# thecasterian/fluca

Hardware: AMD Instinct MI355X
Metric: pressure-Poisson Jacobi-PCG iterations/s, 512^3 cells per GPU (higher is better)
Workload: dtype f64

## Files before the change

fluca_amd/csrc/fl_cheb2.hip:

```cpp
#include <type_traits>

#include "fl_device.h"
#include "fl_handle.h"

namespace fl {

typedef double v2d_t __attribute__((ext_vector_type(2)));
template <int NT>
__device__ __forceinline__ double2 c2_ld2(const double *p)
{
  if (NT) {
    const v2d_t v = __builtin_nontemporal_load(reinterpret_cast<const v2d_t *>(p));
    return make_double2(v.x, v.y);
  }
  return *reinterpret_cast<const double2 *>(p);
}
template <int NT>
__device__ __forceinline__ void c2_st2(double *p, double2 v)
{
  if (NT) {
    v2d_t t;
    t.x = v.x;
    t.y = v.y;
    __builtin_nontemporal_store(t, reinterpret_cast<v2d_t *>(p));
// ... 24 lines not shown
}

__device__ __forceinline__ int c2_xcd_remap(int b, int nblocks) { return (nblocks & 7) ? b : (b & 7) * (nblocks >> 3) + (b >> 3); }

template <int RY, int NW, bool JAC, int NT, bool MGD = false, int Z = 0>
__global__ void __launch_bounds__(64 * NW) k_cheb2(GridP g, int perx, int pery, int perz, const double *X0, const double *X1, double *X0w, double *X1w, const double *__restrict__ b, const double *D0, const double *D1, double *D0w,
                                                  double *D1w, const KspScal *__restrict__ s, double *__restrict__ partial, int stride, int zc, int tiles_x, int tiles, int remap, const double *__restrict__ zq = nullptr,
                                                  const double *__restrict__ za_dev = nullptr, double *__restrict__ bw = nullptr)
{
  constexpr bool ZR = Z != 0, ZS = Z == 2;
  static_assert(!(ZR && MGD), "the three-step sweep is the pre-smoother: no sums of the outer iteration");
  constexpr int TX = 128, TY = NW * RY, LX = TX + 4, NTH = 64 * NW;
  constexpr int NTL = NT >= 2, NTS = NT >= 1;
  __shared__ __attribute__((aligned(16))) double XJ[3][TY + 4][LX];
  __shared__ __attribute__((aligned(16))) double XN[3][TY + 2][LX];
  __shared__ double                              red[6 * NW], cB[2 * TY][5];
  if (s->reason != 0) return;

  const double *x  = s->cur ? X1 : X0;
  double       *xn = s->cur ? X0w : X1w;
  const double *d  = s->dcur ? D1 : D0;
  double       *dn = s->dcur ? D0w : D1w;
  double        rho0 = s->cheb_rho, c0 = s->cheb_c;
  double        rho1, c1;
  const double  cf = s->cheb_c;
  const double  za = ZS ? *za_dev : 0.;
  {
    double ck, ckm1;
    cheb_advance(s, s->ck, s->ckm1, ck, ckm1, rho1, c1);
    if (ZR) {
      rho0 = rho1;
      c0   = c1;
      double ck2, ckm2;
      cheb_advance(s, ck, ckm1, ck2, ckm2, rho1, c1);
    }
  }

  const int bb    = remap ? c2_xcd_remap(blockIdx.x, gridDim.x) : blockIdx.x;
  const int chunk = bb / tiles, tile = bb % tiles;
  const int i0 = (tile % tiles_x) * TX, j0 = (tile / tiles_x) * TY;
// ... 140 lines not shown
        R.hxB = c2_LD1(hx, HB.off);
        R.hbB = c2_LD1(hb, HB.off);
        R.hdB = c2_LD1(hd, HB.off);
      }
      if (anyE) R.hxE = c2_LD1(hx, HE.off);
    }
    R.zcw = ZR ? g.sc[2][pk] : 0.;
    R.pl  = pl;
    const int kz = min(max(kk, -1), g.nz);
    R.zl  = g.sl[2][kz];
    R.zc  = g.sc[2][kz];
    R.zh  = g.sh[2][kz];
    R.pin = pin;
  };

  double  acc[6] = {0., 0., 0., 0., 0., 0.};
  double2 sb2[RY], d1p[RY];
  double2 zb1[RY], zb1R = make_double2(0., 0.);
  double  zb1B = 0.;
  double  z1l = 0., z1c = 0., z1h = 0., z2l = 0., z2c = 0., z2h = 0.;
  bool    pin1 = false;
#pragma unroll
  for (int m = 0; m < RY; ++m) sb2[m] = d1p[m] = zb1[m] = make_double2(0., 0.);

  auto step = [&](auto do1, auto do2, int kk, Raw &C, Raw &N) {
    constexpr bool DO1 = decltype(do1)::value, DO2 = decltype(do2)::value;
    load(kk + 1, N);
    double2 zbn[RY], zbnR = make_double2(0., 0.);
    double  zbnB = 0.;
    if constexpr (ZR) {
      const bool ownk = kk >= k0 && kk < k1;
// ... 99 lines not shown
      if (anyB) {
        const double cen = XJ[bc][HB.lr][HB.lc], dyz = cB[tbc][4] + z1c;
        const double v = dyz * cen + cB[tbc][0] * XJ[bc][HB.lr][HB.lc - 1] + cB[tbc][1] * XJ[bc][HB.lr][HB.lc + 1] + cB[tbc][2] * XJ[bc][HB.lr - 1][HB.lc] + cB[tbc][3] * XJ[bc][HB.lr + 1][HB.lc] + z1l * XJ[bp][HB.lr][HB.lc] + z1h * C.hxB;
        const double r = (ZR ? zb1B : C.hbB) - v, z = JAC ? r / dyz : r;
        const double e = (rho0 != 0. ? rho0 * (ZR ? cen : C.hdB) : 0.) + c0 * z;
        hx1B = (HB.in && pin1) ? cen + e : 0.;
      }
    }

    if constexpr (DO2) {
      const int     bc = (k2 + 3) % 3, bp = (k2 + 2) % 3;
      const int64_t p2 = (int64_t)k2 * g.sxy;
#pragma unroll
      for (int m = 0; m < RY; ++m) {
        const int     lr    = w * RY + m + 1;
        const double2 cen   = *reinterpret_cast<const double2 *>(&XN[bc][lr][lc]);
        const double2 south = *reinterpret_cast<const double2 *>(&XN[bc][lr - 1][lc]);
        const double2 north = *reinterpret_cast<const double2 *>(&XN[bc][lr + 1][lc]);
        const double2 below = *reinterpret_cast<const double2 *>(&XN[bp][lr][lc]);
        const double  west = XN[bc][lr][lc - 1], east = XN[bc][lr][lc + 2];
        const double  dyz = yc[m] + z2c;
        const double  v0 = (xc0 + dyz) * cen.x + xl0 * west + xh0 * cen.y + yl[m] * south.x + yh[m] * north.x + z2l * below.x + z2h * x1v[m].x;
        const double  v1 = (xc1 + dyz) * cen.y + xl1 * cen.x + xh1 * east + yl[m] * south.y + yh[m] * north.y + z2l * below.y + z2h * x1v[m].y;
        const double  r0 = sb2[m].x - v0, r1 = sb2[m].y - v1;
        const double  z0 = JAC ? r0 / (xc0 + dyz) : r0, z1 = JAC ? r1 / (xc1 + dyz) : r1;
        double2       e, xo;
        e.x  = rho1 * d1p[m].x + c1 * z0;
        e.y  = rho1 * d1p[m].y + c1 * z1;
        xo.x = cen.x + e.x;
        xo.y = cen.y + e.y;
        if (rin[m] && in0) {
          if (in1) {
            c2_ST2<NTS>(dn + rob[m] + p2, lo, e);
            c2_ST2<NTS>(xn + rob[m] + p2, lo, xo);
            if (MGD) {
              acc[0] += xo.x + xo.y;
              acc[1] += xo.x * xo.x + xo.y * xo.y;
              acc[2] += sb2[m].x * xo.x + sb2[m].y * xo.y;
              acc[3] += sb2[m].x + sb2[m].y;
              acc[4] += sb2[m].x * sb2[m].x + sb2[m].y * sb2[m].y;
            } else {
              acc[3] += z0 + z1;
              acc[4] += z0 * z0 + z1 * z1;
              acc[5] += r0 * r0 + r1 * r1;
            }
          } else {
            c2_ST1(dn + rob[m] + p2, lo, e.x);
            c2_ST1(xn + rob[m] + p2, lo, xo.x);
            if (MGD) {
              acc[0] += xo.x;
              acc[1] += xo.x * xo.x;
              acc[2] += sb2[m].x * xo.x;
              acc[3] += sb2[m].x;
              acc[4] += sb2[m].x * sb2[m].x;
            } else {
              acc[3] += z0;
              acc[4] += z0 * z0;
              acc[5] += r0 * r0;
            }
          }
        }
      }
    }

    {
      const int bj = (kk + 3) % 3, bn = (kc + 3) % 3;
#pragma unroll
      for (int m = 0; m < RY; ++m) {
        if (rin[m]) {
// ... 46 lines not shown
    using F = std::false_type;
    Raw A, B;
    __syncthreads();
    load(k0 - 2, A);
    step(F(), F(), k0 - 2, A, B);
    step(F(), F(), k0 - 1, B, A);
    step(T(), F(), k0, A, B);
    step(T(), F(), k0 + 1, B, A);
    for (int kk = k0 + 2; kk <= k1 + 1; kk += 2) {
      step(T(), T(), kk, A, B);
      if (kk + 1 <= k1 + 1) step(T(), T(), kk + 1, B, A);
    }
  }

#pragma unroll
  for (int a = 0; a < 6; ++a) {
    acc[a] = wave_sum(acc[a]);
    if (lane == 0) red[a * NW + w] = acc[a];
  }
  __syncthreads();
  if (tid == 0) {
#pragma unroll
    for (int a = 0; a < 6; ++a) {
      double t = 0.;
#pragma unroll
      for (int q = 0; q < NW; ++q) t += red[a * NW + q];
      partial[(int64_t)a * stride + blockIdx.x] = t;
    }
  }
}

}

using namespace fl;


bool fl_cheb2_usable(const fl_poisson *h)
{
// ... 59 lines not shown
    } else {
      if (jac) cheb2_t<4, true, false, 2>(h, p, X0, X1, B, D0, D1, subq, suba_dev, Bw);
      else cheb2_t<4, false, false, 2>(h, p, X0, X1, B, D0, D1, subq, suba_dev, Bw);
    }
    return;
  }
  if (p.nw == 8) {
    if (jac) cheb2_t<8, true, false, 1>(h, p, X0, X1, B, D0, D1);
    else cheb2_t<8, false, false, 1>(h, p, X0, X1, B, D0, D1);
  } else {
    if (jac) cheb2_t<4, true, false, 1>(h, p, X0, X1, B, D0, D1);
    else cheb2_t<4, false, false, 1>(h, p, X0, X1, B, D0, D1);
  }
}

void fl_launch_cheb2(fl_poisson *h, const Cheb2Plan &p, bool jac, double *X0, double *X1, const double *B, double *D0, double *D1, bool mgdots)
{
  if (mgdots) {
    if (p.nw == 8) cheb2_t<8, true, true>(h, p, X0, X1, B, D0, D1);
    else cheb2_t<4, true, true>(h, p, X0, X1, B, D0, D1);
    return;
  }
  if (p.nw == 8) {
    if (jac) cheb2_t<8, true>(h, p, X0, X1, B, D0, D1);
    else cheb2_t<8, false>(h, p, X0, X1, B, D0, D1);
  } else {
    if (jac) cheb2_t<4, true>(h, p, X0, X1, B, D0, D1);
    else cheb2_t<4, false>(h, p, X0, X1, B, D0, D1);
  }
}
```

fluca_amd/csrc/fl_handle.h:

```cpp
#pragma once
#include <algorithm>
#include <cmath>
#include <cstdlib>
#include <cstring>
#include <limits>
#include <list>
#include <string>

#include "fl_internal.h"
#include "fl_knobs.h"

typedef struct ncclComm *ncclComm_t;

namespace fl {

void launch_pad_copy(hipStream_t, const GridP &, const double *, double *);
void launch_unpad_copy(hipStream_t, const GridP &, const double *, double *, const double *);
void launch_project_all(hipStream_t, const GridP &, const double *p, double *const v[3], double *const V[3]);
bool project_six_usable(const GridP &, const double *p_unpadded, double *const v[3], double *const V[3]);
void launch_project_six(hipStream_t, const GridP &, const double *p, bool direct, int per, double *const v[3], double *const V[3]);
void launch_wrap(hipStream_t, const GridP &, double *, int axis, int nvec = 1, int64_t vstride = 0);
void launch_pack_faces_sr(hipStream_t, const GridP &, const double *r, const double *sb, const double *W, const KspScal *s, double *const bufs[6]);
void launch_face_ext(hipStream_t, const GridP &, double *v, double *buf, int axis, int side, int ea, int eb, int mode);
void launch_face_ext_deep(hipStream_t, const GridP &, double *v, double *buf, int axis, int side, int ea, int eb, int dp, int mode);
// ... 74 lines not shown
  int  exchange(hipStream_t st, const std::vector<Msg> &m);
  int  allreduce(hipStream_t st, double *dev, int n);
  void destroy_oneshot();
  void destroy();
};

}

using namespace fl;


struct fl_mg;

struct SmoothSeq {
  int                  nu = 0;
  bool                 guess_zero = false, jac = false, fuse = false, want = false, zero3 = false;
  double               emin = 0., emax = 0.;
  std::vector<KspScal> host;
  KspScal             *dev = nullptr;
};

struct fl_poisson {
  int         device = 0;
  hipStream_t stream = nullptr, own_stream = nullptr;
  Axis        ax[3];
  int         bc[6];
  double      kappa = 0.;
  fl_decomp   dec;
  int         nbr[6];
  bool        wrap_local[3];
  bool        multi = false;
// ... 101 lines not shown
int  fl_fill_ghosts_deep(fl_poisson *h, double *v);
int  fl_fill_hifaces(fl_poisson *h, const double *const V[3]);
int  fl_exchange_r_begin(fl_poisson *h, double *r, const double *q);
int  fl_exchange_sr_begin(fl_poisson *h, const double *r, const double *sb, const double *W, double *rn);
int  fl_exchange_r_end(fl_poisson *h, double *r);
bool fl_any_ghost_exchange(const fl_poisson *h);
int fl_allreduce_max(fl_poisson *h, double *v);
int fl_allreduce_sum(fl_poisson *h, double *v);
int fl_poll_scal(fl_poisson *h);
int fl_apply_tiled(fl_poisson *h, const double *xpad, double *y, int unpadded_y);
int fl_residual(fl_poisson *h, const double *x, const double *b, double *r);
int fl_residual_padded(fl_poisson *h, double *xpad, const double *bpad, double *rpad);
bool fl_residual_restrict_fusable(const GridP &g);
int fl_residual_restrict_padded(fl_poisson *h, double *xpad, const double *bpad, const double *wx, const double *wy, const double *wz, fl_poisson *hc, double *cpad);
int fl_apply_padded_dot(fl_poisson *h, double *xpad, double *ypad, double *xy);
int fl_cheb_smooth_padded(fl_poisson *h, int nu, bool jac, bool guess_zero, bool *mgdots = nullptr, const double *subq = nullptr, const double *suba_dev = nullptr);
int fl_solve_cg(fl_poisson *h, const double *b, double *x, const fl_ksp_opts *o, fl_ksp_stats *st);
int fl_solve_bcgs(fl_poisson *h, const double *b, double *x, const fl_ksp_opts *o, fl_ksp_stats *st);
int fl_solve_cg_sr(fl_poisson *h, const double *b, double *x, const fl_ksp_opts *o, fl_ksp_stats *st);
int fl_ksp_begin(fl_poisson *h, const fl_ksp_opts *o);
int fl_bcgs_fin_step(fl_poisson *h, int mode, int nblocks, int nslot, int nhist);
int fl_ksp_finish(fl_poisson *h, const fl_ksp_opts *o, fl_ksp_stats *st);
int fl_cheb_begin(fl_poisson *h, const fl_ksp_opts *o, double emin, double emax);
int fl_cheb_fin_step(fl_poisson *h, int nblocks, int nhist);
int fl_solve_cheb(fl_poisson *h, const double *b, double *x, const fl_ksp_opts *o, fl_ksp_stats *st);
double fl_gershgorin_bound(const fl_poisson *h, bool jac);
struct Cheb2Plan {
  int nw, tiles_x, tiles, nchunk, zc, nblocks;
};
bool      fl_cheb2_usable(const fl_poisson *h);
int       fl_cheb2_agree(fl_poisson *h);
Cheb2Plan fl_cheb2_plan(const GridP &g);
void      fl_launch_cheb2(fl_poisson *h, const Cheb2Plan &p, bool jac, double *X0, double *X1, const double *B, double *D0, double *D1, bool mgdots = false);
namespace fl {
struct SchurVarT {
  const double *w0[3], *w1[3];
  const int    *c0[3];
};
}
bool      fl_schur_var_usable(const fl_poisson *h);
int       fl_schur_var_fill_ghosts(fl_poisson *h, double *p_pad);
int       fl_schur_var_apply_fused(fl_poisson *h, const fl::SchurVarT &t, const double *ainv, const double *p_pad, double *y);
struct SchurVarPlan {
  int     per_xcd, nseg, band, fixed_seg;
  int64_t items;
};
SchurVarPlan schur_var_plan(const fl::GridP &g);
struct TP {
// ... 8 lines not shown
```

fluca_amd/csrc/fl_internal.h:

```cpp
#pragma once
#include <hip/hip_runtime.h>

#include <algorithm>
#include <cstdint>
#include <cstdio>
#include <vector>

#include "../../include/fluca_hip.h"

#define FL_HIP(call)                                                                                          \
  do {                                                                                                        \
    hipError_t e_ = (call);                                                                                   \
    if (e_ != hipSuccess) {                                                                                   \
      std::fprintf(stderr, "[flucahip] %s:%d %s -> %s\n", __FILE__, __LINE__, #call, hipGetErrorString(e_)); \
      return FL_ERR_GPU;                                                                                      \
    }                                                                                                         \
  } while (0)

#define FL_CHK(call)          \
  do {                        \
    int rc_ = (call);         \
    if (rc_ != 0) return rc_; \
  } while (0)

// ... 56 lines not shown
  R.v[1]    = P1;
  return R;
}

struct KspScal {
  double rz, rz_old, pq, alpha, beta, zshift, dp, rnorm0, ttol;
  double aring[CG_XRING_MAX];
  double rtol, atol, dtol;
  double ncell_global;
  double rho, rho_old, omega, omega_old, d1, d2, vshift, tshift, rshift;
  double ck, ckm1, mu, omegaprod, scale, xshift, dshift, cheb_rho, cheb_c;
  int    it, maxit, reason, norm_type, nullspace, pending_x, cur;
  int    x_valid;
  int    dcur;
  int    xdepth;
};

constexpr int MAX_PARTIAL_BLOCKS = 4096;
constexpr int NSLOT              = 8;

inline int z_chunk_count(int tiles, int nz, int target_blocks, int min_zc = 8)
{
  const int nchunk = std::min(std::max(1, (target_blocks + tiles / 2) / tiles), std::max(1, nz / min_zc));
  return std::max(1, std::min(nchunk, nz));
}
struct ZChunks {
  int nchunk, zc;
};
inline ZChunks z_chunks(int nz, int nchunk)
{
// ... 21 lines not shown
```

fluca_amd/csrc/fl_knobs.h:

```cpp
#pragma once
#include <atomic>

#define FL_PUBLIC_KNOBS(X)                                                                                                                   \
  X(cheb_fuse, 1)                   \
  X(placement, 0)                           \
  X(cg_xbatch, 1)                                           \
  X(cg_xdepth, 8)                 \
  X(cheb_zero3, 1)                  \
  X(mg_prolong, 1)                                                             \
  X(mg_flexible, 1)                                                             \
  X(mg_coarse, 1)                                   \
  X(mg_post_smooth, 0)               \
  X(schur_var_fused, 1)      \
  X(overlap, 1)              \
  X(comm_loopback, 0)           \
  X(comm_trace, 0)                             \
  X(ghost_width, 0)                                       \
  X(placement_verbose, 0)                                                                        \
  X(placement_vmm, 1)                    \
  X(allreduce, 0)

namespace fl {

enum Knob : int {
#define X(n, d) K_##n,
  FL_PUBLIC_KNOBS(X)
#undef X
// ... 10 lines not shown
```

fluca_amd/csrc/fl_ksp.hip:

```cpp
#include <ctime>
#include "fl_handle.h"
#include "fl_device.h"
#include "fl_stencil.h"

namespace fl {

__device__ __forceinline__ double2 LD2(const double *base, unsigned byteoff) { return *reinterpret_cast<const double2 *>(reinterpret_cast<const char *>(base) + byteoff); }
__device__ __forceinline__ void    ST2(double *base, unsigned byteoff, double2 v) { *reinterpret_cast<double2 *>(reinterpret_cast<char *>(base) + byteoff) = v; }
__device__ __forceinline__ void    ST1(double *base, unsigned byteoff, double v) { *reinterpret_cast<double *>(reinterpret_cast<char *>(base) + byteoff) = v; }
__device__ __forceinline__ double uniform(double v)
{
  const int lo = __builtin_amdgcn_readfirstlane(__double2loint(v)), hi = __builtin_amdgcn_readfirstlane(__double2hiint(v));
  return __hiloint2double(hi, lo);
}


struct Tile {
  int  i, il, k0, k1, lane, w, j0w, i0;
  bool own0, own1;
};
template <int RY>
__device__ __forceinline__ Tile make_tile(const GridP &g, int nchunk, int zc, int tiles_x)
{
  Tile      t;
// ... 194 lines not shown
  static constexpr int NACC = MODE == 9 ? 7 : 4;
  static constexpr bool ZST = MODE == 9 || MODE == 10;
};
template <int RY, int NW, bool JAC, int MODE>
__device__ __forceinline__ void st_body(const GridP &g, const double *__restrict__ stg, const double *e0, const double *e1, const double *e2, double *w0, double *w1 ,
                                        const KspScal *__restrict__ s, double *__restrict__ partial, int stride, int nchunk, int zc, int tiles_x, int tiles, int remap, StAux ax = StAux())
{
  static_assert(MODE != 11 || RY == 2, "the restricted residual pairs the two rows of a wave");
  using T               = TileA<RY, NW>;
  constexpr int TX = T::TX, TY = T::TY, LX = T::LX, LY = T::LY;
  constexpr int NE = BcgsIo<MODE>::NE, NACC = BcgsIo<MODE>::NACC;
  constexpr bool ZST = BcgsIo<MODE>::ZST;
  __shared__ __attribute__((aligned(16))) double lds[3][LY][LX];
  __shared__ double                              red[NACC * NW];
  double alpha = 0., omega = 0., beta = 0., ob = 0., vsh = 0., ssh = 0., tsh = 0., crho = 0., cc = 0., zsh = 0.;
  if (MODE < 7 || MODE == 9 || MODE == 10) {
    if (s->reason != 0) return;
    alpha = s->alpha; omega = s->omega; beta = s->beta; ob = s->omega_old * s->beta; vsh = s->vshift; ssh = s->rshift; tsh = s->tshift;
    crho = s->cheb_rho; cc = s->cheb_c; zsh = s->zshift;
  }

  const int b     = remap ? xcd_remap(blockIdx.x, gridDim.x) : blockIdx.x;
  const int chunk = b / tiles, tile = b % tiles;
  const int i0 = (tile % tiles_x) * TX, j0 = (tile / tiles_x) * TY;
  const int k0 = chunk * zc, k1 = min(k0 + zc, g.nz);
  const int tid = threadIdx.x, lane = tid & 63;
  const int w  = __builtin_amdgcn_readfirstlane(tid >> 6);
  const int i  = i0 + 2 * lane;
  const int jb = j0 + w * RY;

  const bool   own0 = i < g.nx, own1 = i + 1 < g.nx;
  const int    il  = min(i, g.nx & ~1);
  const int    ic0 = min(i, g.nx), ic1 = min(i + 1, g.nx);
  const double xl0 = g.sl[0][ic0], xc0 = g.sc[0][ic0], xh0 = g.sh[0][ic0];
// ... 169 lines not shown
          const double  wyz = e2[min(jb + m, g.ny - 1)] * reinterpret_cast<const double *>(w1)[kc];
          racc += wyz * (rwx0 * (ov.x - y.x) + rwx1 * (ov.y - y.y));
          if (m == RY - 1 && (kc & 1)) {
            if (o1) w0[ax.coff + (int64_t)(kc >> 1) * ax.csxy + (int64_t)(jb >> 1) * ax.csx + (i >> 1)] = racc;
            racc = 0.;
          }
        } else if (MODE == 6) {
          const double2 bv = C.e[0][m], dv = C.e[NE >= 2 ? 1 : 0][m];
          const double  r0 = bv.x - y.x, r1 = bv.y - y.y;
          const double  z0 = JAC ? r0 / (xc0 + dyc) : r0, z1 = JAC ? r1 / (xc1 + dyc) : r1;
          double2       dn, xo;
          dn.x = (crho != 0. ? crho * dv.x : 0.) + cc * z0;
          dn.y = (crho != 0. ? crho * dv.y : 0.) + cc * z1;
          xo.x = cen.x + dn.x;
          xo.y = cen.y + dn.y;
          put(w1, dn);
          put(w0, xo);
          acc[0] += (o0 ? z0 : 0.) + (o1 ? z1 : 0.);
          acc[1] += (o0 ? z0 * z0 : 0.) + (o1 ? z1 * z1 : 0.);
          acc[2] += (o0 ? r0 * r0 : 0.) + (o1 ? r1 * r1 : 0.);
        } else {
          const double2 R = C.e[0][m];
          double2       o;
          o.x = R.x - ob * (y.x - vsh) + beta * cen.x;
          o.y = R.y - ob * (y.y - vsh) + beta * cen.y;
          put(w0, o);
        }
      }
    }
#pragma unroll
    for (int m = 0; m < RY; ++m) {
// ... 172 lines not shown
  s->pq     = dpi;
  s->beta   = b;
  s->alpha  = betan / dpi;
}

template <int RY, bool JAC>
__global__ void __launch_bounds__(256) k_cheb(GridP g, const double *X0, const double *X1, double *X0w, double *X1w, const double *__restrict__ b, double *D0, double *D1,
                                              const KspScal *__restrict__ s, double *__restrict__ partial, int stride, int nchunk, int zc, int tiles_x)
{
  __shared__ double red[3 * 4];
  if (s->reason != 0) return;
  const double *x  = s->cur ? X1 : X0;
  double       *xn = s->cur ? X0w : X1w;
  double *__restrict__ d = s->dcur ? D1 : D0;
  const double  rho = s->cheb_rho, cc = s->cheb_c;
  const Tile    t = make_tile<RY>(g, nchunk, zc, tiles_x);
  const double  xl0 = g.sl[0][min(t.i, g.nx)], xc0 = g.sc[0][min(t.i, g.nx)], xh0 = g.sh[0][min(t.i, g.nx)];
  const double  xl1 = g.sl[0][min(t.i + 1, g.nx)], xc1 = g.sc[0][min(t.i + 1, g.nx)], xh1 = g.sh[0][min(t.i + 1, g.nx)];
  double        acc[3] = {0., 0., 0.};
  if (t.k0 < t.k1) {
    double2       prev[RY], cur[RY], nxt[RY], so_c, no_c, so_n, no_n;
    double        we_c[RY], ee_c[RY], we_n[RY], ee_n[RY];
    unsigned      lo = 8u * (unsigned)t.il;
    const int     i0 = t.i0;
    const int64_t sxy = g.sxy;
    const int64_t rsou = g.off0 + (int64_t)min(t.j0w - 1, g.ny) * g.sx, rnor = g.off0 + (int64_t)min(t.j0w + RY, g.ny) * g.sx;
    int64_t       rj[RY];
#pragma unroll
    for (int m = 0; m < RY; ++m) rj[m] = g.off0 + (int64_t)min(t.j0w + m, g.ny) * g.sx;
    const int wofs = i0 - 1, eofs = min(i0 + 128, g.nx);
// ... 33 lines not shown
        const double  west = t.lane == 0 ? we_c[m] : up, east = t.lane == 63 ? ee_c[m] : dn;
        const double  dyz = ycc + zcc;
        double2       v;
        v.x = (xc0 + dyz) * cur[m].x + xl0 * west + xh0 * cur[m].y + yl * so.x + yh * no.x + zl * prev[m].x + zh * nxt[m].x;
        v.y = (xc1 + dyz) * cur[m].y + xl1 * cur[m].x + xh1 * east + yl * so.y + yh * no.y + zl * prev[m].y + zh * nxt[m].y;
        if (j < g.ny && t.own0) {
          const bool   two = t.own1;
          const double r0 = bv[m].x - v.x, r1 = two ? bv[m].y - v.y : 0.;
          const double z0 = JAC ? r0 / (xc0 + dyz) : r0, z1 = two ? (JAC ? r1 / (xc1 + dyz) : r1) : 0.;
          double2      dn2, xo;
          dn2.x = (rho != 0. ? rho * dv[m].x : 0.) + cc * z0;
          dn2.y = (rho != 0. ? rho * dv[m].y : 0.) + cc * z1;
          xo.x  = cur[m].x + dn2.x;
          xo.y  = cur[m].y + dn2.y;
          if (two) {
            ST2(d + rj[m] + pc, lo, dn2);
            ST2(xn + rj[m] + pc, lo, xo);
          } else {
            ST1(d + rj[m] + pc, lo, dn2.x);
            ST1(xn + rj[m] + pc, lo, xo.x);
          }
          acc[0] += z0 + z1;
          acc[1] += z0 * z0 + z1 * z1;
          acc[2] += r0 * r0 + r1 * r1;
        }
      }
#pragma unroll
      for (int m = 0; m < RY; ++m) {
        prev[m] = cur[m];
        cur[m]  = nxt[m];
        we_c[m] = uniform(we_n[m]);
        ee_c[m] = uniform(ee_n[m]);
      }
      so_c = so_n;
// ... 366 lines not shown

int fl_apply_padded_dot(fl_poisson *h, double *xpad, double *ypad, double *xy)
{
  FL_CHK(fl_fill_ghosts(h, xpad));
  const PlanA pa = plan_cg_A(h->g, 0, 0);
  FL_CHK(fl_ensure_partials(h, pa.nblocks));
  launch_bcgs_st<7>(h, pa, false, xpad, nullptr, nullptr, nullptr, ypad, nullptr);
  launch_reduce(h->stream, h->partial, pa.nblocks, h->partial_stride, 4, h->sums);
  if (h->multi) FL_CHK(h->comm.allreduce(h->stream, h->sums, NSLOT));
  if (!xy) return 0;
  FL_HIP(hipMemcpyAsync(xy, h->sums + 2, sizeof(double), hipMemcpyDeviceToHost, h->stream));
  FL_HIP(hipStreamSynchronize(h->stream));
  return 0;
}

int fl_cheb_smooth_padded(fl_poisson *h, int nu, bool jac, bool guess_zero, bool *mgdots, const double *subq, const double *suba)
{
  if (subq && !(guess_zero && nu > 0)) return FL_ERR_ARG_WRONGSTATE;
  const bool want = mgdots && *mgdots;
  if (mgdots) *mgdots = false;
  for (double **v : {&h->r, &h->P0, &h->q, &h->xp}) FL_CHK(fl_ensure_vec(h, v));
  if (nu <= 0) {
    if (guess_zero) FL_CHK(fl_zero_vec(h, h->xp));
    return 0;
  }
  const TP tp = tile_plan(h->g);
  FL_CHK(fl_ensure_partials(h, std::max(tp.nblocks, 1024)));
  const int nhist = nu + 2;
  FL_CHK(fl_ensure_hist(h, nhist));
  hipStream_t  s = h->stream;
  fl_ksp_opts  o;
// ... 23 lines not shown
  }
  double    *X0 = h->xp, *X1 = h->P0, *B = h->r, *D0 = h->q, *D1 = fuse ? h->cd1 : h->q;
  const bool ghosts = fl_any_ghost_exchange(h);
  int        cur = 0, dcur = 0;
  const int trace = knob(K_comm_trace);
  auto mark = [&](const char *what, int j) {
    if (!trace) return;
    const bool sync = trace >= 2;
    const hipError_t e = sync ? hipStreamSynchronize(s) : hipSuccess;
    struct timespec ts;
    clock_gettime(CLOCK_MONOTONIC, &ts);
    std::fprintf(stderr, "[%.3f smooth r%d n=%dx%dx%d] %s j=%d cur=%d dcur=%d -> %s\n", ts.tv_sec % 1000 + 1e-9 * ts.tv_nsec, h->comm.rank, h->g.nx, h->g.ny, h->g.nz, what, j, cur, dcur, hipGetErrorString(e));
    std::fflush(stderr);
  };
  const bool zero3 = fuse && guess_zero && nu >= 3 && !h->multi && knob(K_cheb_zero3) != 0;
  auto kind_of = [&](int j) { return (j == 0 && guess_zero) ? (zero3 ? 3 : 1) : ((fuse && j + 2 <= nu && !(want && jac && !h->multi && ((nu - j) & 1))) ? 2 : 0); };
  const KspScal *seq = nullptr;
  {
    SmoothSeq *hit = nullptr;
    for (SmoothSeq &q : h->smooth_seq)
      if (q.nu == nu && q.guess_zero == guess_zero && q.jac == jac && q.fuse == fuse && q.want == want && q.zero3 == zero3 && q.emin == emin && q.emax == emax) hit = &q;
    if (!hit) {
      SmoothSeq q;
      q.nu = nu; q.guess_zero = guess_zero; q.jac = jac; q.fuse = fuse; q.want = want; q.zero3 = zero3; q.emin = emin; q.emax = emax;
      KspScal S = S0;
      auto advance = [](const KspScal &P, double ck, double ckm1, double &ck_out, double &ckm1_out, double &rho, double &c) {
        const double ckp1 = 2. * P.mu * ck - ckm1, omega = P.omegaprod * ck / ckp1;
        ckm1_out = ck;
        ck_out   = ckp1;
        rho      = omega - 1.;
        c        = omega * P.scale;
      };
      for (int j = 0; j < nu;) {
        q.host.push_back(S);
        if (kind_of(j) == 3) {
          double ck, ckm1, ck2, ckm2, rho, c;
          advance(S, S.ck, S.ckm1, ck, ckm1, rho, c);
          advance(S, ck, ckm1, ck2, ckm2, rho, c);
          S.cur ^= 1;
// ... 11 lines not shown
          S.cheb_rho = rho2;
          S.cheb_c   = c2;
          j += 2;
        } else {
          double ck, ckm1, rho, c;
          S.cur ^= 1;
          S.it += 1;
          advance(S, S.ck, S.ckm1, ck, ckm1, rho, c);
          S.ck       = ck;
          S.ckm1     = ckm1;
          S.cheb_rho = rho;
          S.cheb_c   = c;
          j += 1;
        }
      }
      FL_HIP(hipMalloc((void **)&q.dev, sizeof(KspScal) * q.host.size()));
      h->smooth_seq.push_back(std::move(q));
      hit = &h->smooth_seq.back();
      FL_HIP(hipMemcpyAsync(hit->dev, hit->host.data(), sizeof(KspScal) * hit->host.size(), hipMemcpyHostToDevice, s));
    }
    seq = hit->dev;
  }
  struct ScalGuard {
    fl_poisson *h;
    KspScal    *keep;
    ~ScalGuard() { h->scal = keep; }
  } guard{h, h->scal};
  const bool deep = fuse && h->multi;
  bool       bghost = false;
  int        launch = 0;
// ... 19 lines not shown
      if (subq) {
        if (jac) hipLaunchKernelGGL((k_cheb_first<true, true>), dim3(nb), dim3(256), 0, s, h->g, X0, X1, B, D0, D1, h->scal, subq, suba);
        else hipLaunchKernelGGL((k_cheb_first<false, true>), dim3(nb), dim3(256), 0, s, h->g, X0, X1, B, D0, D1, h->scal, subq, suba);
      } else if (jac) hipLaunchKernelGGL((k_cheb_first<true>), dim3(nb), dim3(256), 0, s, h->g, X0, X1, B, D0, D1, h->scal, (const double *)nullptr, (const double *)nullptr);
      else hipLaunchKernelGGL((k_cheb_first<false>), dim3(nb), dim3(256), 0, s, h->g, X0, X1, B, D0, D1, h->scal, (const double *)nullptr, (const double *)nullptr);
      j += 1;
    } else if (kind == 2) {
      const bool md = want && jac && j + 2 == nu && !h->multi;
      if (deep) {
        if (!bghost) FL_CHK(fl_fill_ghosts(h, B));
        bghost = true;
        FL_CHK(fl_fill_ghosts_deep(h, cur ? X1 : X0));
        FL_CHK(fl_fill_ghosts(h, dcur ? D1 : D0));
      }
      mark("ghosts filled, before fused", j);
      fl_launch_cheb2(h, cp, jac, X0, X1, B, D0, D1, md);
      mark("fused done", j);
      dcur ^= 1;
      if (md) {
        launch_reduce(s, h->partial, cp.nblocks, h->partial_stride, 5, h->sums);
        *mgdots = true;
      }
      j += 2;
    } else {
      if (ghosts) FL_CHK(fl_fill_ghosts(h, cur ? X1 : X0));
      mark("before single", j);
      (void)launch_cheb(h, tp, jac, X0, X1, B, D0, D1);
      mark("single done", j);
      j += 1;
    }
    cur ^= 1;
  }
  if (cur) std::swap(h->xp, h->P0);
  h->poisoned = true;
  return 0;
// ... 323 lines not shown
```

fluca_amd/csrc/fl_mg.hip:

```cpp
#include <new>

#include "fl_handle.h"
#include "fl_device.h"

namespace fl {

struct Owned {
  int64_t npair_row, npairs;
};
__device__ __forceinline__ Owned owned_of(const GridP &g)
{
  Owned o;
  o.npair_row = (g.nx + 1) / 2;
  o.npairs    = o.npair_row * (int64_t)g.ny * g.nz;
  return o;
}
__device__ __forceinline__ int64_t pair_off(const GridP &g, const Owned &o, int64_t q, bool &two)
{
  const int     ip = (int)(q % o.npair_row);
  const int64_t row = q / o.npair_row;
  const int     j = (int)(row % g.ny), k = (int)(row / g.ny);
  two = 2 * ip + 1 < g.nx;
  return g.off0 + (int64_t)k * g.sxy + (int64_t)j * g.sx + 2 * ip;
}
// ... 537 lines not shown
    for (double **v : {&hl->r, &hl->P0, &hl->q, &hl->xp}) FL_CHK(fl_ensure_vec(hl, v));
    if (l + 1 == mg->lv.size()) {
      FL_CHK(alloc_cells(hl, &L.x));
      FL_CHK(alloc_cells(hl, &L.b));
    }
    FL_CHK(fl_ensure_partials(hl, MG_BLOCKS));
  }
  for (double **v : {&h->w0, &h->w1, &h->w2}) FL_CHK(fl_ensure_vec(h, v));
  FL_HIP(hipMalloc((void **)&mg->scal, sizeof(MgScal)));
  FL_HIP(hipMalloc((void **)&mg->slot_dev, 2 * sizeof(MgSlot)));
  FL_HIP(hipHostMalloc((void **)&mg->slot_host, 2 * sizeof(MgSlot)));
  for (hipEvent_t &e : mg->ev_slot) FL_HIP(hipEventCreateWithFlags(&e, hipEventDisableTiming));
  return 0;
}

int vcycle(fl_mg *mg, size_t l, const fl_ksp_opts *o, bool *sums = nullptr, const double *subq = nullptr)
{
  const bool want = sums && *sums;
  if (sums) *sums = false;
  MgLevel    &L = mg->lv[l];
  fl_poisson *h = L.h;
  if (l + 1 == mg->lv.size()) {
    fl_ksp_stats st;
    fl_ksp_opts  so;
    fl_ksp_opts_default(&so);
    so.remove_nullspace = o->remove_nullspace;
    so.type  = FL_KSP_CG;
    so.pc    = FL_PC_JACOBI;
    so.rtol  = 1e-2;
    so.maxit = 200;
    if (subq) hipLaunchKernelGGL(k_mg_pwd<5>, dim3(nblk_pairs(h->g)), dim3(256), 0, h->stream, h->g, (const MgScal *)mg->scal, (const double *)nullptr, subq, (double *)nullptr, h->r);
// ... 32 lines not shown
      t.pn[d] = L.pn[d];
      t.pw[d] = L.pw[d];
    }
    if (L.r[0] == 2 && L.r[1] == 2 && L.r[2] == 2) {
      const int  kc = 4;
      const GridP &gcs = C.h->g;
      hipLaunchKernelGGL(k_mg_prolong_lin_cc, dim3((gcs.nx + 61) / 62, (gcs.ny + 3) / 4, (gcs.nz + kc - 1) / kc), dim3(256), 0, h->stream, h->g, gcs, t, (const double *)C.h->xp, h->xp, kc);
    } else {
      const int  zc = 8;
      const dim3 grid((h->g.nx + 127) / 128, (h->g.ny + 3) / 4, (h->g.nz + zc - 1) / zc);
      hipLaunchKernelGGL(k_mg_prolong_lin_tile, grid, dim3(256), 0, h->stream, h->g, C.h->g, L.r[0], L.r[1], L.r[2], t, (const double *)C.h->xp, h->xp, zc);
    }
  } else hipLaunchKernelGGL(k_mg_prolong_add, dim3(nblk_pairs(h->g)), dim3(256), 0, h->stream, h->g, C.h->g, L.r[0], L.r[1], L.r[2], C.h->xp, h->xp);
  bool got = want;
  const int nu_post = knob(K_mg_post_smooth) > 0 ? knob(K_mg_post_smooth) : nu;
  FL_CHK(fl_cheb_smooth_padded(h, nu_post, true, false, &got));
  if (sums) *sums = got;
  return 0;
}

}

void fl_mg_destroy(fl_poisson *h)
{
  fl_mg *mg = h->mg;
  if (!mg) return;
  for (size_t l = 0; l < mg->lv.size(); ++l) {
    MgLevel &L = mg->lv[l];
    for (double *p : {L.x, L.b, L.w[0], L.w[1], L.w[2], L.pw[0], L.pw[1], L.pw[2]})
      if (p) (void)hipFree(p);
    for (int *p : L.pn)
// ... 53 lines not shown
    MgScal init;
    std::memset(&init, 0, sizeof(init));
    init.N      = N;
    init.ns     = ns ? 1 : 0;
    init.pnorm  = pnorm ? 1 : 0;
    init.rz_old = 1.;
    hipLaunchKernelGGL(k_mg_scal_set, dim3(1), dim3(1), 0, s, S, init);
  }
  auto dots_dev = [&](const double *z, const double *r) -> int {
    hipLaunchKernelGGL(k_mg_dots, dim3(nb), dim3(256), 0, s, g, z, r, h->partial, h->partial_stride);
    launch_reduce(s, h->partial, nb, h->partial_stride, 5, h->sums);
    if (h->multi) FL_CHK(h->comm.allreduce(s, h->sums, NSLOT));
    return 0;
  };
  const double *subq = nullptr;
  auto cycle_and_sums = [&](int it, bool first) -> int {
    bool got = true;
    FL_CHK(vcycle(mg, 0, o, &got, subq));
    if (!got) FL_CHK(dots_dev(h->xp, h->r));
    const int a = it & 1;
    if (first) hipLaunchKernelGGL((k_mg_scal<1, true>), dim3(1), dim3(1), 0, s, S, (const double *)h->sums, mg->slot_dev + a);
    else hipLaunchKernelGGL((k_mg_scal<1, false>), dim3(1), dim3(1), 0, s, S, (const double *)h->sums, mg->slot_dev + a);
    FL_HIP(hipMemcpyAsync(mg->slot_host + a, mg->slot_dev + a, sizeof(MgSlot), hipMemcpyDeviceToHost, s));
    FL_HIP(hipEventRecord(mg->ev_slot[a], s));
    return 0;
  };
  auto look = [&](int it) -> int {
    const int a = it & 1;
    FL_HIP(hipEventSynchronize(mg->ev_slot[a]));
    const MgSlot &L = mg->slot_host[a];
    dp     = L.dp;
    rz     = L.rz;
    pq     = L.pq;
// ... 4 lines not shown
  FL_CHK(fl_zero_vec(h, X));
  FL_CHK(cycle_and_sums(0, true));
  hipLaunchKernelGGL(k_mg_pwd<2>, dim3(nb), dim3(256), 0, s, g, (const MgScal *)S, (const double *)h->xp, (const double *)nullptr, P, (double *)nullptr);
  FL_CHK(look(0));
  const double rnorm0 = dp, ttol = std::max(o->rtol * dp, o->atol);
  hist.push_back(dp);
  int  it = 0, reason = 0;
  auto converged = [&](double v) {
    if (std::isnan(v) || std::isinf(v)) return (int)FL_DIVERGED_NANORINF;
    if (v <= ttol) return v < o->atol ? (int)FL_CONVERGED_ATOL : (int)FL_CONVERGED_RTOL;
    if (v >= o->dtol * rnorm0) return (int)FL_DIVERGED_DTOL;
    return 0;
  };
  reason = converged(dp);
  if (!reason && o->maxit <= 0) reason = FL_DIVERGED_ITS;
  const bool flexible = fl_mg_flexible_mode() != 0;
  while (!reason) {
    FL_CHK(fl_apply_padded_dot(h, P, Q, nullptr));
    hipLaunchKernelGGL((k_mg_scal<0>), dim3(1), dim3(1), 0, s, S, (const double *)h->sums, (MgSlot *)nullptr);
    subq = Q;
    FL_CHK(cycle_and_sums(it + 1, false));
    subq = nullptr;
    if (flexible) {
      FL_CHK(dots_dev(h->xp, Q));
      hipLaunchKernelGGL((k_mg_scal<2>), dim3(1), dim3(1), 0, s, S, (const double *)h->sums, (MgSlot *)nullptr);
    } else hipLaunchKernelGGL((k_mg_scal<3>), dim3(1), dim3(1), 0, s, S, (const double *)h->sums, (MgSlot *)nullptr);
    hipLaunchKernelGGL(k_mg_pwd<4>, dim3(nb), dim3(256), 0, s, g, (const MgScal *)S, (const double *)h->xp, (const double *)nullptr, P, X);
    FL_CHK(look(it + 1));
    if (bad_pq) {
      reason = std::isnan(pq) ? FL_DIVERGED_NANORINF : FL_DIVERGED_INDEFINITE_MAT;
      break;
    }
    ++it;
    hist.push_back(dp);
    reason = converged(dp);
    if (!reason && it >= o->maxit) reason = FL_DIVERGED_ITS;
    if (!reason && !(rz > 0.)) reason = std::isnan(rz) ? FL_DIVERGED_NANORINF : FL_DIVERGED_INDEFINITE_PC;
  }
// ... 30 lines not shown
```

Measured before the change: 715.0.

## Fuse flexible-PCG q·z dots into final smoother sweep and skip dead direction store

The last fused Chebyshev post-smoothing sweep now also reads Q and accumulates q·x and sum(q), so the flexible outer PCG can take its extra dot products from the smoother's reduction. This removes a separate dots kernel and reduce pass over two full vectors each iteration. The final smoother step also skips writing the Chebyshev direction vector when it will not be reused, saving one full-grid store. In exchange the sweep does an additional streaming load of Q and reduces two more accumulators.

```diff
diff --git a/fluca_amd/csrc/fl_cheb2.hip b/fluca_amd/csrc/fl_cheb2.hip
--- a/fluca_amd/csrc/fl_cheb2.hip
+++ b/fluca_amd/csrc/fl_cheb2.hip
@@ -62,7 +62,8 @@
   constexpr int NTL = NT >= 2, NTS = NT >= 1;
   __shared__ __attribute__((aligned(16))) double XJ[3][TY + 4][LX];
   __shared__ __attribute__((aligned(16))) double XN[3][TY + 2][LX];
-  __shared__ double                              red[6 * NW], cB[2 * TY][5];
+  constexpr int NA = MGD ? 7 : 6;
+  __shared__ double                              red[NA * NW], cB[2 * TY][5];
   if (s->reason != 0) return;
 
   const double *x  = s->cur ? X1 : X0;
@@ -72,6 +73,7 @@
   double        rho0 = s->cheb_rho, c0 = s->cheb_c;
   double        rho1, c1;
   const double  cf = s->cheb_c;
+  const bool    keepd = s->d_dead == 0;
   const double  za = ZS ? *za_dev : 0.;
   {
     double ck, ckm1;
@@ -242,7 +244,7 @@
     R.pin = pin;
   };
 
-  double  acc[6] = {0., 0., 0., 0., 0., 0.};
+  double  acc[7] = {0., 0., 0., 0., 0., 0., 0.};
   double2 sb2[RY], d1p[RY];
   double2 zb1[RY], zb1R = make_double2(0., 0.);
   double  zb1B = 0.;
@@ -372,6 +374,7 @@
 #pragma unroll
       for (int m = 0; m < RY; ++m) {
         const int     lr    = w * RY + m + 1;
+        const double2 qv = (MGD && zq) ? c2_LD2<NTL>(zq + rob[m] + p2, lo) : make_double2(0., 0.);
         const double2 cen   = *reinterpret_cast<const double2 *>(&XN[bc][lr][lc]);
         const double2 south = *reinterpret_cast<const double2 *>(&XN[bc][lr - 1][lc]);
         const double2 north = *reinterpret_cast<const double2 *>(&XN[bc][lr + 1][lc]);
@@ -389,7 +392,7 @@
         xo.y = cen.y + e.y;
         if (rin[m] && in0) {
           if (in1) {
-            c2_ST2<NTS>(dn + rob[m] + p2, lo, e);
+            if (keepd) c2_ST2<NTS>(dn + rob[m] + p2, lo, e);
             c2_ST2<NTS>(xn + rob[m] + p2, lo, xo);
             if (MGD) {
               acc[0] += xo.x + xo.y;
@@ -397,13 +400,15 @@
               acc[2] += sb2[m].x * xo.x + sb2[m].y * xo.y;
               acc[3] += sb2[m].x + sb2[m].y;
               acc[4] += sb2[m].x * sb2[m].x + sb2[m].y * sb2[m].y;
+              acc[5] += qv.x * xo.x + qv.y * xo.y;
+              acc[6] += qv.x + qv.y;
             } else {
               acc[3] += z0 + z1;
               acc[4] += z0 * z0 + z1 * z1;
               acc[5] += r0 * r0 + r1 * r1;
             }
           } else {
-            c2_ST1(dn + rob[m] + p2, lo, e.x);
+            if (keepd) c2_ST1(dn + rob[m] + p2, lo, e.x);
             c2_ST1(xn + rob[m] + p2, lo, xo.x);
             if (MGD) {
               acc[0] += xo.x;
@@ -411,6 +416,8 @@
               acc[2] += sb2[m].x * xo.x;
               acc[3] += sb2[m].x;
               acc[4] += sb2[m].x * sb2[m].x;
+              acc[5] += qv.x * xo.x;
+              acc[6] += qv.x;
             } else {
               acc[3] += z0;
               acc[4] += z0 * z0;
@@ -487,14 +494,14 @@
   }
 
 #pragma unroll
-  for (int a = 0; a < 6; ++a) {
+  for (int a = 0; a < NA; ++a) {
     acc[a] = wave_sum(acc[a]);
     if (lane == 0) red[a * NW + w] = acc[a];
   }
   __syncthreads();
   if (tid == 0) {
 #pragma unroll
-    for (int a = 0; a < 6; ++a) {
+    for (int a = 0; a < NA; ++a) {
       double t = 0.;
 #pragma unroll
       for (int q = 0; q < NW; ++q) t += red[a * NW + q];
@@ -584,11 +591,11 @@
   }
 }
 
-void fl_launch_cheb2(fl_poisson *h, const Cheb2Plan &p, bool jac, double *X0, double *X1, const double *B, double *D0, double *D1, bool mgdots)
+void fl_launch_cheb2(fl_poisson *h, const Cheb2Plan &p, bool jac, double *X0, double *X1, const double *B, double *D0, double *D1, bool mgdots, const double *dotq)
 {
   if (mgdots) {
-    if (p.nw == 8) cheb2_t<8, true, true>(h, p, X0, X1, B, D0, D1);
-    else cheb2_t<4, true, true>(h, p, X0, X1, B, D0, D1);
+    if (p.nw == 8) cheb2_t<8, true, true>(h, p, X0, X1, B, D0, D1, dotq);
+    else cheb2_t<4, true, true>(h, p, X0, X1, B, D0, D1, dotq);
     return;
   }
   if (p.nw == 8) {
diff --git a/fluca_amd/csrc/fl_handle.h b/fluca_amd/csrc/fl_handle.h
--- a/fluca_amd/csrc/fl_handle.h
+++ b/fluca_amd/csrc/fl_handle.h
@@ -112,7 +112,7 @@
 
 struct SmoothSeq {
   int                  nu = 0;
-  bool                 guess_zero = false, jac = false, fuse = false, want = false, zero3 = false;
+  bool                 guess_zero = false, jac = false, fuse = false, want = false, zero3 = false, keep_d = false;
   double               emin = 0., emax = 0.;
   std::vector<KspScal> host;
   KspScal             *dev = nullptr;
@@ -244,7 +244,7 @@
 bool fl_residual_restrict_fusable(const GridP &g);
 int fl_residual_restrict_padded(fl_poisson *h, double *xpad, const double *bpad, const double *wx, const double *wy, const double *wz, fl_poisson *hc, double *cpad);
 int fl_apply_padded_dot(fl_poisson *h, double *xpad, double *ypad, double *xy);
-int fl_cheb_smooth_padded(fl_poisson *h, int nu, bool jac, bool guess_zero, bool *mgdots = nullptr, const double *subq = nullptr, const double *suba_dev = nullptr);
+int fl_cheb_smooth_padded(fl_poisson *h, int nu, bool jac, bool guess_zero, bool *mgdots = nullptr, const double *subq = nullptr, const double *suba_dev = nullptr, const double *dotq = nullptr);
 int fl_solve_cg(fl_poisson *h, const double *b, double *x, const fl_ksp_opts *o, fl_ksp_stats *st);
 int fl_solve_bcgs(fl_poisson *h, const double *b, double *x, const fl_ksp_opts *o, fl_ksp_stats *st);
 int fl_solve_cg_sr(fl_poisson *h, const double *b, double *x, const fl_ksp_opts *o, fl_ksp_stats *st);
@@ -261,7 +261,7 @@
 bool      fl_cheb2_usable(const fl_poisson *h);
 int       fl_cheb2_agree(fl_poisson *h);
 Cheb2Plan fl_cheb2_plan(const GridP &g);
-void      fl_launch_cheb2(fl_poisson *h, const Cheb2Plan &p, bool jac, double *X0, double *X1, const double *B, double *D0, double *D1, bool mgdots = false);
+void      fl_launch_cheb2(fl_poisson *h, const Cheb2Plan &p, bool jac, double *X0, double *X1, const double *B, double *D0, double *D1, bool mgdots = false, const double *dotq = nullptr);
 namespace fl {
 struct SchurVarT {
   const double *w0[3], *w1[3];
diff --git a/fluca_amd/csrc/fl_internal.h b/fluca_amd/csrc/fl_internal.h
--- a/fluca_amd/csrc/fl_internal.h
+++ b/fluca_amd/csrc/fl_internal.h
@@ -94,6 +94,7 @@
   int    x_valid;
   int    dcur;
   int    xdepth;
+  int    d_dead;
 };
 
 constexpr int MAX_PARTIAL_BLOCKS = 4096;
diff --git a/fluca_amd/csrc/fl_knobs.h b/fluca_amd/csrc/fl_knobs.h
--- a/fluca_amd/csrc/fl_knobs.h
+++ b/fluca_amd/csrc/fl_knobs.h
@@ -11,6 +11,8 @@
   X(mg_flexible, 1)                                                             \
   X(mg_coarse, 1)                                   \
   X(mg_post_smooth, 0)               \
+  X(smooth_keep_d, 0)        \
+  X(mg_outer_fused, 1)     \
   X(schur_var_fused, 1)      \
   X(overlap, 1)              \
   X(comm_loopback, 0)           \
diff --git a/fluca_amd/csrc/fl_ksp.hip b/fluca_amd/csrc/fl_ksp.hip
--- a/fluca_amd/csrc/fl_ksp.hip
+++ b/fluca_amd/csrc/fl_ksp.hip
@@ -232,10 +232,12 @@
   __shared__ __attribute__((aligned(16))) double lds[3][LY][LX];
   __shared__ double                              red[NACC * NW];
   double alpha = 0., omega = 0., beta = 0., ob = 0., vsh = 0., ssh = 0., tsh = 0., crho = 0., cc = 0., zsh = 0.;
+  bool   keepd = true;
   if (MODE < 7 || MODE == 9 || MODE == 10) {
     if (s->reason != 0) return;
     alpha = s->alpha; omega = s->omega; beta = s->beta; ob = s->omega_old * s->beta; vsh = s->vshift; ssh = s->rshift; tsh = s->tshift;
     crho = s->cheb_rho; cc = s->cheb_c; zsh = s->zshift;
+    if (MODE == 6) keepd = s->d_dead == 0;
   }
 
   const int b     = remap ? xcd_remap(blockIdx.x, gridDim.x) : blockIdx.x;
@@ -435,7 +437,7 @@
           dn.y = (crho != 0. ? crho * dv.y : 0.) + cc * z1;
           xo.x = cen.x + dn.x;
           xo.y = cen.y + dn.y;
-          put(w1, dn);
+          if (keepd) put(w1, dn);
           put(w0, xo);
           acc[0] += (o0 ? z0 : 0.) + (o1 ? z1 : 0.);
           acc[1] += (o0 ? z0 * z0 : 0.) + (o1 ? z1 * z1 : 0.);
@@ -638,6 +640,7 @@
   double       *xn = s->cur ? X0w : X1w;
   double *__restrict__ d = s->dcur ? D1 : D0;
   const double  rho = s->cheb_rho, cc = s->cheb_c;
+  const bool    keepd = s->d_dead == 0;
   const Tile    t = make_tile<RY>(g, nchunk, zc, tiles_x);
   const double  xl0 = g.sl[0][min(t.i, g.nx)], xc0 = g.sc[0][min(t.i, g.nx)], xh0 = g.sh[0][min(t.i, g.nx)];
   const double  xl1 = g.sl[0][min(t.i + 1, g.nx)], xc1 = g.sc[0][min(t.i + 1, g.nx)], xh1 = g.sh[0][min(t.i + 1, g.nx)];
@@ -701,10 +704,10 @@
           xo.x  = cur[m].x + dn2.x;
           xo.y  = cur[m].y + dn2.y;
           if (two) {
-            ST2(d + rj[m] + pc, lo, dn2);
+            if (keepd) ST2(d + rj[m] + pc, lo, dn2);
             ST2(xn + rj[m] + pc, lo, xo);
           } else {
-            ST1(d + rj[m] + pc, lo, dn2.x);
+            if (keepd) ST1(d + rj[m] + pc, lo, dn2.x);
             ST1(xn + rj[m] + pc, lo, xo.x);
           }
           acc[0] += z0 + z1;
@@ -1101,7 +1104,7 @@
   return 0;
 }
 
-int fl_cheb_smooth_padded(fl_poisson *h, int nu, bool jac, bool guess_zero, bool *mgdots, const double *subq, const double *suba)
+int fl_cheb_smooth_padded(fl_poisson *h, int nu, bool jac, bool guess_zero, bool *mgdots, const double *subq, const double *suba, const double *dotq)
 {
   if (subq && !(guess_zero && nu > 0)) return FL_ERR_ARG_WRONGSTATE;
   const bool want = mgdots && *mgdots;
@@ -1155,15 +1158,16 @@
     std::fflush(stderr);
   };
   const bool zero3 = fuse && guess_zero && nu >= 3 && !h->multi && knob(K_cheb_zero3) != 0;
+  const bool keep_d = knob(K_smooth_keep_d) != 0;
   auto kind_of = [&](int j) { return (j == 0 && guess_zero) ? (zero3 ? 3 : 1) : ((fuse && j + 2 <= nu && !(want && jac && !h->multi && ((nu - j) & 1))) ? 2 : 0); };
   const KspScal *seq = nullptr;
   {
     SmoothSeq *hit = nullptr;
     for (SmoothSeq &q : h->smooth_seq)
-      if (q.nu == nu && q.guess_zero == guess_zero && q.jac == jac && q.fuse == fuse && q.want == want && q.zero3 == zero3 && q.emin == emin && q.emax == emax) hit = &q;
+      if (q.nu == nu && q.guess_zero == guess_zero && q.jac == jac && q.fuse == fuse && q.want == want && q.zero3 == zero3 && q.keep_d == keep_d && q.emin == emin && q.emax == emax) hit = &q;
     if (!hit) {
       SmoothSeq q;
-      q.nu = nu; q.guess_zero = guess_zero; q.jac = jac; q.fuse = fuse; q.want = want; q.zero3 = zero3; q.emin = emin; q.emax = emax;
+      q.nu = nu; q.guess_zero = guess_zero; q.jac = jac; q.fuse = fuse; q.want = want; q.zero3 = zero3; q.keep_d = keep_d; q.emin = emin; q.emax = emax;
       KspScal S = S0;
       auto advance = [](const KspScal &P, double ck, double ckm1, double &ck_out, double &ckm1_out, double &rho, double &c) {
         const double ckp1 = 2. * P.mu * ck - ckm1, omega = P.omegaprod * ck / ckp1;
@@ -1205,6 +1209,7 @@
           j += 1;
         }
       }
+      q.host.back().d_dead = keep_d ? 0 : 1;
       FL_HIP(hipMalloc((void **)&q.dev, sizeof(KspScal) * q.host.size()));
       h->smooth_seq.push_back(std::move(q));
       hit = &h->smooth_seq.back();
@@ -1254,11 +1259,11 @@
         FL_CHK(fl_fill_ghosts(h, dcur ? D1 : D0));
       }
       mark("ghosts filled, before fused", j);
-      fl_launch_cheb2(h, cp, jac, X0, X1, B, D0, D1, md);
+      fl_launch_cheb2(h, cp, jac, X0, X1, B, D0, D1, md, md ? dotq : nullptr);
       mark("fused done", j);
       dcur ^= 1;
       if (md) {
-        launch_reduce(s, h->partial, cp.nblocks, h->partial_stride, 5, h->sums);
+        launch_reduce(s, h->partial, cp.nblocks, h->partial_stride, dotq ? 7 : 5, h->sums);
         *mgdots = true;
       }
       j += 2;
diff --git a/fluca_amd/csrc/fl_mg.hip b/fluca_amd/csrc/fl_mg.hip
--- a/fluca_amd/csrc/fl_mg.hip
+++ b/fluca_amd/csrc/fl_mg.hip
@@ -575,7 +575,7 @@
   return 0;
 }
 
-int vcycle(fl_mg *mg, size_t l, const fl_ksp_opts *o, bool *sums = nullptr, const double *subq = nullptr)
+int vcycle(fl_mg *mg, size_t l, const fl_ksp_opts *o, bool *sums = nullptr, const double *subq = nullptr, const double *dotq = nullptr)
 {
   const bool want = sums && *sums;
   if (sums) *sums = false;
@@ -638,7 +638,7 @@
   } else hipLaunchKernelGGL(k_mg_prolong_add, dim3(nblk_pairs(h->g)), dim3(256), 0, h->stream, h->g, C.h->g, L.r[0], L.r[1], L.r[2], C.h->xp, h->xp);
   bool got = want;
   const int nu_post = knob(K_mg_post_smooth) > 0 ? knob(K_mg_post_smooth) : nu;
-  FL_CHK(fl_cheb_smooth_padded(h, nu_post, true, false, &got));
+  FL_CHK(fl_cheb_smooth_padded(h, nu_post, true, false, &got, nullptr, nullptr, dotq));
   if (sums) *sums = got;
   return 0;
 }
@@ -722,9 +722,13 @@
     return 0;
   };
   const double *subq = nullptr;
+  const bool    flexible = fl_mg_flexible_mode() != 0;
+  const double *dotq = nullptr;
+  bool          qsums = false;
   auto cycle_and_sums = [&](int it, bool first) -> int {
     bool got = true;
-    FL_CHK(vcycle(mg, 0, o, &got, subq));
+    FL_CHK(vcycle(mg, 0, o, &got, subq, dotq));
+    qsums = got && dotq;
     if (!got) FL_CHK(dots_dev(h->xp, h->r));
     const int a = it & 1;
     if (first) hipLaunchKernelGGL((k_mg_scal<1, true>), dim3(1), dim3(1), 0, s, S, (const double *)h->sums, mg->slot_dev + a);
@@ -759,14 +763,17 @@
   };
   reason = converged(dp);
   if (!reason && o->maxit <= 0) reason = FL_DIVERGED_ITS;
-  const bool flexible = fl_mg_flexible_mode() != 0;
+  const bool ride = flexible && !h->multi && knob(K_mg_outer_fused) != 0;
   while (!reason) {
     FL_CHK(fl_apply_padded_dot(h, P, Q, nullptr));
     hipLaunchKernelGGL((k_mg_scal<0>), dim3(1), dim3(1), 0, s, S, (const double *)h->sums, (MgSlot *)nullptr);
     subq = Q;
+    dotq = ride ? Q : nullptr;
     FL_CHK(cycle_and_sums(it + 1, false));
-    subq = nullptr;
-    if (flexible) {
+    subq = dotq = nullptr;
+    if (flexible && qsums) {
+      hipLaunchKernelGGL((k_mg_scal<2>), dim3(1), dim3(1), 0, s, S, (const double *)h->sums + 3, (MgSlot *)nullptr);
+    } else if (flexible) {
       FL_CHK(dots_dev(h->xp, Q));
       hipLaunchKernelGGL((k_mg_scal<2>), dim3(1), dim3(1), 0, s, S, (const double *)h->sums, (MgSlot *)nullptr);
     } else hipLaunchKernelGGL((k_mg_scal<3>), dim3(1), dim3(1), 0, s, S, (const double *)h->sums, (MgSlot *)nullptr);
```

After: 715.2 (median of 2 runs). No clear change (+0.0%).
